# hpc4cmb/flacarray

Hardware: AMD Instinct MI355X
Metric: Msamples/s encode+decode, 4096ch x 1Msamp int32 (higher is better)
Workload: dtype int32

## Files before the change

flacarray_amd/csrc/decode_kernels.hpp:

```cpp
#pragma once
#include <hip/hip_runtime.h>
#include <stdint.h>

#include <type_traits>
#include <utility>

#include "flac_math.hpp"
#include "quantize_kernels.hpp"

namespace fa {

constexpr int kErrDecodeInit = 1 << 13;
constexpr int kErrDecodeProcess = 1 << 14;
constexpr int kErrDecodeSeek = 1 << 18;

constexpr int64_t kFrameUnset = -2;
constexpr int kScanSpan = 256 * 16;

struct StreamMeta {
    int64_t first_frame;
    int64_t seek_abs;
    int64_t end_abs;
    int32_t npoints;
    int32_t B;
// ... 372 lines not shown
            } else ok = false;
            if (ok && pred) {
                const int method = (int)br.get(2);
                const int po = (int)br.get(4);
                const int plen = method ? 5 : 4, esc = method ? 31 : 15;
                if (method > 1 || order > h.bs) ok = false;
                const int ps = h.bs >> po;
                for (int p = 0; ok && p < (1 << po); ++p) {
                    const int n = (p == 0) ? ps - order : ps;
                    if (n < 0) { ok = false; break; }
                    const int k = (int)br.get(plen);
                    if (k == esc) {
                        const int nbw = (int)br.get(5);
                        br.skip((int64_t)nbw * n);
                    } else {
                        for (int j = 0; j < n; ++j) {
                            const uint32_t q = br.unary();
                            if (q > (1u << 24)) { ok = false; break; }
                            if (k) br.get(k);
                        }
                    }
                }
            }
        }
        if (!ok) { atomicOr(err, kErrDecodeProcess); for (int64_t r = f + 1; r < nf; ++r) ftab[s * nf + r] = -1; return; }
        const int64_t bits = (br.used + 7) & ~(int64_t)7;
        at += (bits >> 3) + 2;
    }
    (void)stream_size;
}

struct DecodeArgs {
    const uint8_t* blob;
    int64_t blob_bytes;
    const StreamMeta* meta;
    const int64_t* ftab;
    int64_t nf;
    int32_t B;
    int64_t stream_size;
    int64_t n_tasks;
    int64_t nfr;
    int64_t f0;
    int64_t first;
    int64_t n_decode;
    const int64_t* task_stream;
    const int64_t* task_frame;
    const int64_t* task_first;
    const int64_t* task_last;
    const int64_t* task_out_off;
    union { int32_t* out_i32; long long* red_min; };
    union { float* out_f32; long long* red_max; };
    union { const float* offsets; long long* red_sum; };
    union { const float* gains; unsigned long long* red_sq_hi; };
    int* err;
    union { uint32_t* hibits; unsigned long long* red_sq_lo; };
    int32_t* assign;
    int32_t hib_words;
    int32_t verbatim_done;
    union { const void* cmp; int64_t red_width; };
    union { unsigned long long* first_mismatch; int64_t red_nbins; };
};

template <int... U, class F>
__device__ __forceinline__ void static_for_impl(std::integer_sequence<int, U...>, F&& f) {
    (f(std::integral_constant<int, U>{}), ...);
}
template <int N, class F>
__device__ __forceinline__ void static_for(F&& f) {
    static_for_impl(std::make_integer_sequence<int, N>{}, static_cast<F&&>(f));
}

#ifndef FA_TILE_W
#define FA_TILE_W 32
#endif
#ifndef FA_K7_SPEC
#define FA_K7_SPEC 0
#endif
#ifndef FA_K7_SEED
#define FA_K7_SEED 0
#endif
#ifndef FA_K7_NT
#define FA_K7_NT 1
#endif
#ifndef FA_K7_X
#define FA_K7_X 0
#endif
constexpr int kTileW = FA_TILE_W;
constexpr int kTileG = kTileW / 4;
constexpr int kTileSwz = 32 / kTileG;
#ifndef FA_CHUNK_BYTES
#define FA_CHUNK_BYTES 64
#endif
constexpr int kChunkBytes = FA_CHUNK_BYTES;
constexpr int kChunkW = kChunkBytes / 4;
constexpr int kChunkShift = (kChunkBytes == 64) ? 9 : 8;
constexpr int kRingW = 2 * kChunkW;
constexpr int kDecRingWords = kRingW + 2;
constexpr int kTopup = kChunkBytes / 8;
constexpr int kLaneStride = 64;

constexpr int kFlagNeed16 = 1, kFlagNeed32 = 2;
__device__ __forceinline__ int4 shl4(const int4& v, int n) {
    return make_int4((int)((uint32_t)v.x << n), (int)((uint32_t)v.y << n), (int)((uint32_t)v.z << n), (int)((uint32_t)v.w << n));
}

__device__ __forceinline__ void ring_load_chunk(const uint8_t* cbase, const uint8_t* lim16, uint32_t* ring, uint32_t ci) {
    const uint8_t* q = cbase + (size_t)ci * kChunkBytes;
    uint32_t* dst = ring + (ci & 1) * kChunkW * kLaneStride;
#pragma unroll
    for (int v = 0; v < kChunkBytes / 16; ++v) {
        uint4 d = make_uint4(0, 0, 0, 0);
        if (q + 16 * v + 16 <= lim16) d = *reinterpret_cast<const uint4*>(q + 16 * v);
        d.x = __builtin_bswap32(d.x); d.y = __builtin_bswap32(d.y); d.z = __builtin_bswap32(d.z); d.w = __builtin_bswap32(d.w);
        dst[(4 * v + 0) * kLaneStride] = d.x; dst[(4 * v + 1) * kLaneStride] = d.y;
        dst[(4 * v + 2) * kLaneStride] = d.z; dst[(4 * v + 3) * kLaneStride] = d.w;
        if (v == 0 && (ci & 1) == 0) { ring[kRingW * kLaneStride] = d.x; ring[(kRingW + 1) * kLaneStride] = d.y; }
    }
}
struct Chunk {
    uint4 d[kChunkBytes / 16];
};
__device__ __forceinline__ Chunk chunk_fetch(const uint8_t* cbase, const uint8_t* lim16, uint32_t ci) {
    const uint8_t* q = cbase + (size_t)ci * kChunkBytes;
    Chunk c;
#pragma unroll
    for (int v = 0; v < kChunkBytes / 16; ++v) {
        c.d[v] = make_uint4(0, 0, 0, 0);
#if (FA_K7_X & 8)
        c.d[v] = make_uint4(0x55555555u ^ ci, 0x55555555u, 0x55555555u, 0x55555555u);
#else
        if (q + 16 * v + 16 <= lim16) c.d[v] = *reinterpret_cast<const uint4*>(q + 16 * v);
#endif
    }
    return c;
}
__device__ __forceinline__ void chunk_store(uint32_t* ring, uint32_t ci, const Chunk& c) {
    uint32_t* dst = ring + (ci & 1) * kChunkW * kLaneStride;
#pragma unroll
    for (int v = 0; v < kChunkBytes / 16; ++v) {
        uint4 d = c.d[v];
        d.x = __builtin_bswap32(d.x); d.y = __builtin_bswap32(d.y); d.z = __builtin_bswap32(d.z); d.w = __builtin_bswap32(d.w);
        dst[(4 * v + 0) * kLaneStride] = d.x; dst[(4 * v + 1) * kLaneStride] = d.y;
        dst[(4 * v + 2) * kLaneStride] = d.z; dst[(4 * v + 3) * kLaneStride] = d.w;
        if (v == 0 && (ci & 1) == 0) { ring[kRingW * kLaneStride] = d.x; ring[(kRingW + 1) * kLaneStride] = d.y; }
    }
}
typedef __attribute__((address_space(3))) uint32_t lds_u32;
constexpr uint32_t kRingAddrMask = (uint32_t)(kRingW - 1) << 8;
__device__ __forceinline__ void ring_words(uint32_t lane4, uint32_t bitpos, uint32_t& w0, uint32_t& w1, uint32_t& w2) {
    static_assert(kLaneStride == 64, "word wi of a lane lies 256 wi bytes behind its word 0");
    uint32_t t, ad;
    asm("v_add_lshl_u32 %0, %2, -1, 3\n\tv_and_or_b32 %1, %0, %3, %4" : "=&v"(t), "=v"(ad) : "v"(bitpos), "s"(kRingAddrMask), "v"(lane4));
    const lds_u32* p = (const lds_u32*)(uintptr_t)ad;
    w0 = p[0]; w1 = p[kLaneStride]; w2 = p[2 * kLaneStride];
}
__device__ __forceinline__ uint32_t ring_word3(uint32_t lane4, uint32_t bitpos, uint32_t k95) {
    uint32_t t, ad;
    asm("v_add_lshl_u32 %0, %2, %5, 3\n\tv_and_or_b32 %1, %0, %3, %4" : "=&v"(t), "=v"(ad) : "v"(bitpos), "s"(kRingAddrMask), "v"(lane4), "s"(k95));
    return *(const lds_u32*)(uintptr_t)ad;
}
__device__ __forceinline__ void ring_window(const uint32_t* ring, uint32_t bitpos, uint32_t& A, uint32_t& B) {
    const uint32_t wi = (bitpos >> 5) & (kRingW - 1);
    const uint32_t off = bitpos & 31;
    uint32_t w0 = ring[wi * kLaneStride], w1 = ring[(wi + 1) * kLaneStride], w2 = ring[(wi + 2) * kLaneStride];
    asm volatile("" : "+v"(w0), "+v"(w1), "+v"(w2));
    A = (uint32_t)((((((uint64_t)w0) << 32) | w1) << off) >> 32);
// ... 65 lines not shown
        o.escw = r.val;
    }
    o.bitpos = r.bitpos;
    o.next_chunk = ring_ensure(cbase, lim16, ring, r.bitpos, r.next_chunk);
    return o;
}
__device__ __noinline__ BitsRet slow_sample(const uint8_t* cbase, const uint8_t* lim16, uint32_t* ring, uint32_t bitpos,
                                            uint32_t next_chunk, int k, int escw) {
    BitsRet r;
    if (escw > 0) {
        r = slow_get(cbase, lim16, ring, bitpos, next_chunk, escw);
        r.val = (uint32_t)((int32_t)(r.val << (32 - escw)) >> (32 - escw));
    } else {
        const BitsRet q = slow_unary(cbase, lim16, ring, bitpos, next_chunk);
        r = slow_get(cbase, lim16, ring, q.bitpos, q.next_chunk, k);
        const uint32_t uu = (q.val << k) | r.val;
        r.val = (uint32_t)((int32_t)(uu >> 1) ^ -(int32_t)(uu & 1));
        r.bad = q.bad;
    }
    r.next_chunk = ring_ensure(cbase, lim16, ring, r.bitpos, r.next_chunk);
    return r;
}

#define FA_GET(n) ({ const BitsRet r_ = slow_get(cbase, lim16, ring, bitpos, next_chunk, (n)); bitpos = r_.bitpos; next_chunk = r_.next_chunk; r_.val; })
#define FA_GETS(n) ({ const int n_ = (n); const uint32_t v_ = FA_GET(n_); (n_ == 0) ? 0 : ((int32_t)(v_ << (32 - n_)) >> (32 - n_)); })
#define FA_UNARY() ({ const BitsRet r_ = slow_unary(cbase, lim16, ring, bitpos, next_chunk); bitpos = r_.bitpos; next_chunk = r_.next_chunk; if (r_.bad) bad = true; r_.val; })

template <int MO, int MO_DONE, bool F32, int NCH, bool CMP = false, bool RED = false>
#ifndef FA_K7_WAVES_ATTR
#define FA_K7_WAVES_ATTR
#endif
__global__ __launch_bounds__(64) FA_K7_WAVES_ATTR void decode_frames_kernel(DecodeArgs a, int* flags) {
    constexpr int kTileW = (NCH == 1 && MO <= 16) ? FA_TILE_W : 32;
    constexpr int kTileG = kTileW / 4;
    constexpr int kTileSwz = 32 / kTileG;
    static_assert(NCH == 1 || (kTileW == 32 && !F32), "two-channel variant: 32-sample tiles, integer output");
    static_assert(!RED || (NCH == 1 && !F32 && !CMP), "reducing sink: one channel, integer domain");
    constexpr bool SINK = CMP && NCH == 1;
    __shared__ __attribute__((aligned(16))) uint32_t lds_k7[kDecRingWords * kLaneStride + (RED ? 0 : kTileW * kLaneStride) + (F32 ? 128 : 0)];
    uint32_t* const rings = lds_k7;
    int32_t* const tile = reinterpret_cast<int32_t*>(lds_k7 + kDecRingWords * kLaneStride);
    float2* const row_fg = reinterpret_cast<float2*>(lds_k7 + kDecRingWords * kLaneStride + kTileW * kLaneStride);
    const int lane = threadIdx.x;
    const int64_t task = (int64_t)blockIdx.x * 64 + lane;
    const bool has_task = task < a.n_tasks;
    uint32_t* const ring = rings + lane;
    const uint32_t lane4 = (uint32_t)(uintptr_t)(lds_u32*)ring;
    if ((uint32_t)(uintptr_t)(lds_u32*)rings & (kRingAddrMask | 255u)) {
        if (lane == 0) atomicOr(a.err, kErrDecodeInit);
        return;
    }

    int64_t s = 0, f = 0, sl_first = 0, sl_last = 0, out_off = 0;
    if (has_task) {
        if (a.task_stream) {
            s = a.task_stream[task]; f = a.task_frame[task];
            sl_first = a.task_first[task]; sl_last = a.task_last[task];
            out_off = a.task_out_off[task];
        } else {
            s = task / a.nfr; f = a.f0 + (task - s * a.nfr);
            sl_first = a.first; sl_last = a.first + a.n_decode;
            if constexpr (RED) out_off = s * a.red_nbins;
            else out_off = s * a.n_decode;
        }
    }
    const int64_t fstart = f * (int64_t)a.B;
    auto reject = [&]() __attribute__((always_inline)) {
        if constexpr (CMP) atomicMin(a.first_mismatch + s, (unsigned long long)fstart);
        else atomicOr(a.err, kErrDecodeProcess);
    };
    const uint8_t* cbase = a.blob;
    const uint8_t* const lim16 = reinterpret_cast<const uint8_t*>((reinterpret_cast<uintptr_t>(a.blob + a.blob_bytes) + 15) & ~(uintptr_t)15);
    uint32_t bitpos = 0, next_chunk = 0x00400000u;

    bool bad = false;
    bool task_live = has_task;
    int fbs = 0, fbps = 0, ch_assign = 0, si_bps = 0;
    if (has_task) {
        const StreamMeta m = a.meta[s];
        si_bps = m.bps;
        const int64_t at = a.ftab[s * a.nf + f];
        if (m.first_frame < 0 || at < 0) bad = true;
        else {
            const uint8_t* start = a.blob + at;
            cbase = reinterpret_cast<const uint8_t*>(reinterpret_cast<uintptr_t>(start - 1) & ~(uintptr_t)(kChunkBytes - 1));
            if (cbase < a.blob) cbase = a.blob;
            bitpos = (uint32_t)(start - cbase) * 8;
            ring_load_chunk(cbase, lim16, ring, 0);
            ring_load_chunk(cbase, lim16, ring, 1);
            next_chunk = 2;
            {
                uint8_t c8 = 0;
                const uint32_t w = FA_GET(32);
                c8 = crc8_byte(c8, (uint8_t)(w >> 24));
                c8 = crc8_byte(c8, (uint8_t)(w >> 16));
                c8 = crc8_byte(c8, (uint8_t)(w >> 8));
                c8 = crc8_byte(c8, (uint8_t)w);
                if ((w >> 16) != 0xFFF8) bad = true;
                const uint32_t b2 = (w >> 8) & 0xff, b3 = w & 0xff;
                const int bsc = (int)(b2 >> 4), src = (int)(b2 & 15), ch = (int)(b3 >> 4), ssc = (int)((b3 >> 1) & 7);
                if (!channel_code_ok(ch, NCH) || (b3 & 1)) bad = true;
                ch_assign = ch;
                const uint32_t u0 = FA_GET(8);
                c8 = crc8_byte(c8, (uint8_t)u0);
                int extra = 0;
                if (u0 & 0x80) {
                    int mbit = 0x40;
                    while ((u0 & mbit) && extra < 7) { extra++; mbit >>= 1; }
                    if (extra == 0 || extra > 6) bad = true;
                }
                for (int i = 0; i < extra && !bad; ++i) c8 = crc8_byte(c8, (uint8_t)FA_GET(8));
                if (bsc == 0) bad = true;
                else if (bsc == 1) fbs = 192;
                else if (bsc <= 5) fbs = 576 << (bsc - 2);
                else if (bsc == 6) { const uint32_t v = FA_GET(8); c8 = crc8_byte(c8, (uint8_t)v); fbs = (int)v + 1; }
                else if (bsc == 7) { const uint32_t v = FA_GET(16); c8 = crc8_byte(c8, (uint8_t)(v >> 8)); c8 = crc8_byte(c8, (uint8_t)v); fbs = (int)v + 1; }
                else fbs = 256 << (bsc - 8);
                if (src == 12) { c8 = crc8_byte(c8, (uint8_t)FA_GET(8)); }
                else if (src == 13 || src == 14) { const uint32_t v = FA_GET(16); c8 = crc8_byte(c8, (uint8_t)(v >> 8)); c8 = crc8_byte(c8, (uint8_t)v); }
                else if (src == 15) bad = true;
                if (FA_GET(8) != c8) bad = true;
                switch (ssc) {
                    case 0: fbps = si_bps; break;
                    case 1: fbps = 8; break;
                    case 2: fbps = 12; break;
                    case 4: fbps = 16; break;
                    case 5: fbps = 20; break;
                    case 6: fbps = 24; break;
                    case 7: fbps = 32; break;
                    default: bad = true; break;
                }
            }
            int64_t expect = a.stream_size - fstart;
            if (expect > a.B) expect = a.B;
            if (fbs != (int)expect) bad = true;
        }
        if constexpr (NCH == 2) {
            if (a.assign[task] >= 0) task_live = false;
        }
        if (bad) { task_live = false; reject(); }
    }
    const void* const out_base = SINK ? a.cmp : (a.out_f32 ? (const void*)a.out_f32 : (const void*)a.out_i32);
    const bool out_aligned = ((reinterpret_cast<uintptr_t>(out_base) & 15) == 0);

    auto get_wide = [&](int n) __attribute__((always_inline)) -> double {
        if constexpr (NCH == 2) {
            if (n > 32) {
                const uint32_t top = FA_GET(1);
                const uint32_t low = FA_GET(32);
                return (double)low - (top ? 4294967296.0 : 0.0);
            }
        }
        return (double)FA_GETS(n);
    };
    auto wrap32 = [&](double v) __attribute__((always_inline)) -> int32_t {
        if constexpr (NCH == 2) {
            if (v >= 2147483648.0) v -= 4294967296.0;
            else if (v < -2147483648.0) v += 4294967296.0;
        }
        return (int32_t)v;
    };

#pragma unroll 1
    for (int chn = 0; chn < NCH; ++chn) {
    int lo = 0, hi = 0;
    int bs = 0;
    int mode = 3;
    int order = 0, bps = 0, wasted = 0;
    double cval = 0.0;
    double scale = 1.0;
// ... 465 lines not shown
#endif
                } else {
#if (FA_K7_X & 2)
                    if (v.x == 0x12345678)
#endif
#if FA_K7_NT
                    {
                        typedef int i32x4_t __attribute__((ext_vector_type(4)));
                        i32x4_t vv; vv.x = v.x; vv.y = v.y; vv.z = v.z; vv.w = v.w;
                        __builtin_nontemporal_store(vv, reinterpret_cast<i32x4_t*>(a.out_i32 + rout[it] + tbase + cb));
                    }
#else
                    *reinterpret_cast<int4*>(a.out_i32 + rout[it] + tbase + cb) = v;
#endif
                }
            }
            __builtin_amdgcn_wave_barrier();
            return;
        }
#pragma unroll
        for (int it = 0; it < kTileG; ++it) {
            const int r = it * kRowsPerPass + (lane / kTileG);
            const int cg = lane % kTileG;
            const int cb = 4 * cg;
            const int rsw = r ^ (cg * kTileSwz);
            int4 v = make_int4(tile[(cb + 0) * kLaneStride + rsw], tile[(cb + 1) * kLaneStride + rsw], tile[(cb + 2) * kLaneStride + rsw],
                               tile[(cb + 3) * kLaneStride + rsw]);
            if (__builtin_expect(any_wasted, 0)) v = shl4(v, __builtin_amdgcn_ds_bpermute(r << 2, wasted));
            const int2 rg = make_int2(__builtin_amdgcn_ds_bpermute(r << 2, lo), __builtin_amdgcn_ds_bpermute(r << 2, hi));
            const int si = tbase + cb;
            int jd = 4;
            if (si + 3 >= rg.x && si < rg.y) {
                const int64_t ob = rout[it] + si;
                const bool fullv = (si >= rg.x) && (si + 3 < rg.y) && out_aligned && ((ob & 3) == 0);
                if constexpr (SINK) {
                    if (fullv) {
                        const int4 x = input4(ob, r);
                        jd = (v.x != x.x) ? 0 : (v.y != x.y) ? 1 : (v.z != x.z) ? 2 : (v.w != x.w) ? 3 : 4;
                    } else {
                        if (si + 3 >= rg.x && si + 3 < rg.y && input1(ob + 3, r) != v.w) jd = 3;
                        if (si + 2 >= rg.x && si + 2 < rg.y && input1(ob + 2, r) != v.z) jd = 2;
                        if (si + 1 >= rg.x && si + 1 < rg.y && input1(ob + 1, r) != v.y) jd = 1;
                        if (si + 0 >= rg.x && si + 0 < rg.y && input1(ob + 0, r) != v.x) jd = 0;
                    }
                } else if constexpr (F32) {
                    const float2 fg = row_fg[r];
                    float4 o;
                    o.x = __fadd_rn(fg.x, __fmul_rn(fg.y, (float)v.x));
                    o.y = __fadd_rn(fg.x, __fmul_rn(fg.y, (float)v.y));
                    o.z = __fadd_rn(fg.x, __fmul_rn(fg.y, (float)v.z));
                    o.w = __fadd_rn(fg.x, __fmul_rn(fg.y, (float)v.w));
                    if (fullv) *reinterpret_cast<float4*>(a.out_f32 + ob) = o;
                    else {
                        if (si + 0 >= rg.x && si + 0 < rg.y) a.out_f32[ob + 0] = o.x;
                        if (si + 1 >= rg.x && si + 1 < rg.y) a.out_f32[ob + 1] = o.y;
                        if (si + 2 >= rg.x && si + 2 < rg.y) a.out_f32[ob + 2] = o.z;
                        if (si + 3 >= rg.x && si + 3 < rg.y) a.out_f32[ob + 3] = o.w;
                    }
                } else {
                    if (fullv) *reinterpret_cast<int4*>(a.out_i32 + ob) = v;
                    else {
                        if (si + 0 >= rg.x && si + 0 < rg.y) a.out_i32[ob + 0] = v.x;
                        if (si + 1 >= rg.x && si + 1 < rg.y) a.out_i32[ob + 1] = v.y;
                        if (si + 2 >= rg.x && si + 2 < rg.y) a.out_i32[ob + 2] = v.z;
                        if (si + 3 >= rg.x && si + 3 < rg.y) a.out_i32[ob + 3] = v.w;
                    }
                }
            }
            if constexpr (SINK) report(r, rout[it] + si, jd);
        }
        __builtin_amdgcn_wave_barrier();
    };

    const int bs_max = a.B;
    constexpr int MACRO = kTileW;
    static_assert(MACRO % MO == 0 && MACRO % 16 == 0, "history rotation and tile must divide the macro step");
    auto macro_step = [&](auto guard_tag, auto part_tag, int i0) __attribute__((always_inline)) {
        static_for<MACRO>([&](auto ut) __attribute__((always_inline)) {
            constexpr int u = decltype(ut)::value;
            const int i = i0 + u;
            if constexpr ((u % kTopup) == 0) {
                topup();
            }
            sample(guard_tag, part_tag, ut, i);
            if constexpr (u == MACRO - 1) flush_tile(i0);
        });
    };
    constexpr int kStep = (MACRO > kTileW) ? MACRO : kTileW;
    int end = (bs_max + kStep - 1) / kStep * kStep;
    if (chn == NCH - 1) {
        const int need = (hi_max + kStep - 1) / kStep * kStep;
        if (need < end) end = need;
    }
    if constexpr (NCH == 2) {
        if (!__any(mode != 3)) end = 0;
    }
    int main_lo = (32 + MACRO - 1) / MACRO * MACRO;
    if (main_lo > end) main_lo = end;
    int main_hi = (bs_min < bs_max ? bs_min : bs_max) / MACRO * MACRO;
    if (main_hi > end) main_hi = end;
    if (main_hi < main_lo) main_hi = main_lo;
    for (int pass = 0; pass < 2; ++pass) {
        const int g_lo = pass == 0 ? 0 : main_hi;
        const int g_hi = pass == 0 ? main_lo : end;
        for (int i0 = g_lo; i0 < g_hi; i0 += MACRO) macro_step(std::true_type{}, std::true_type{}, i0);
        if (pass == 0) {
            for (int i0 = main_lo; i0 < main_hi; i0 += MACRO) {
                if (__any(pleft < MACRO)) {
                    macro_step(std::false_type{}, std::true_type{}, i0);
                } else {
                    macro_step(std::false_type{}, std::false_type{}, i0);
                    pleft -= MACRO;
                }
            }
        }
    }
    if constexpr (NCH == 2) {
        if (skipped) {
            bitpos = resume_bitpos;
            next_chunk = ring_ensure(cbase, lim16, ring, bitpos, bitpos >> kChunkShift);
        }
    }
    }
    if constexpr (NCH == 2) {
        if (has_task && task_live) a.assign[task] = ch_assign;
    }
}

__global__ __launch_bounds__(256) void verbatim_channel0_kernel(DecodeArgs a) {
    const int64_t task = blockIdx.x;
    int64_t s, f, sl_first, sl_last;
    if (a.task_stream) {
        s = a.task_stream[task]; f = a.task_frame[task];
        sl_first = a.task_first[task]; sl_last = a.task_last[task];
    } else {
        s = task / a.nfr; f = a.f0 + (task - s * a.nfr);
        sl_first = a.first; sl_last = a.first + a.n_decode;
    }
    const StreamMeta m = a.meta[s];
    const int64_t at = a.ftab[s * a.nf + f];
    if (m.first_frame < 0 || at < 0 || at + 5 > a.blob_bytes) return;
    const uint8_t* const p = a.blob + at;
    const uint32_t b2 = p[2], b3 = p[3], u0 = p[4];
    const int bsc = (int)(b2 >> 4), src = (int)(b2 & 15), ch = (int)(b3 >> 4), ssc = (int)((b3 >> 1) & 7);
    if (p[0] != 0xFF || p[1] != 0xF8 || (ch != 1 && ch != 8 && ch != 9 && ch != 10)) return;
    int extra = 0;
    if (u0 & 0x80) {
        int mbit = 0x40;
        while ((u0 & mbit) && extra < 7) { extra++; mbit >>= 1; }
        if (extra == 0 || extra > 6) return;
    }
    const int hl = 4 + 1 + extra + (bsc == 6 ? 1 : bsc == 7 ? 2 : 0) + (src == 12 ? 1 : (src == 13 || src == 14) ? 2 : 0) + 1;
    if (at + hl + 1 > a.blob_bytes || p[hl] != 0x02) return;
    int fbps;
    switch (ssc) {
        case 0: fbps = m.bps; break;
        case 1: fbps = 8; break;
        case 2: fbps = 12; break;
        case 4: fbps = 16; break;
        case 5: fbps = 20; break;
        case 6: fbps = 24; break;
        case 7: fbps = 32; break;
        default: return;
    }
    const int bps = fbps + (ch == 9 ? 1 : 0);
    if (bps <= 0 || bps > 33) return;
    const int64_t fstart = f * (int64_t)a.B;
    int64_t bs = a.stream_size - fstart;
    if (bs > a.B) bs = a.B;
    int64_t lo = sl_first - fstart, hi = sl_last - fstart;
    if (lo < 0) lo = 0;
    if (hi > bs) hi = bs;
    if (hi <= lo) return;
    int32_t* const t0 = a.out_i32 + (task * 2 + 0) * (int64_t)a.B;
    uint32_t* const h0 = a.hibits + (task * 2 + 0) * (int64_t)a.hib_words;
    const uint64_t bit0 = 8ull * (uint64_t)(hl + 1);
    const int lane = threadIdx.x & 63;
    const int64_t i0 = lo & ~(int64_t)31;
    const int64_t i1 = ((hi + 31) & ~(int64_t)31) < ((bs + 31) & ~(int64_t)31) ? ((hi + 31) & ~(int64_t)31) : ((bs + 31) & ~(int64_t)31);
    for (int64_t i = i0 + threadIdx.x; i < i1; i += 256) {
        uint32_t low = 0;
        bool neg = false;
        if (i < bs) {
            const uint64_t bp = bit0 + (uint64_t)i * (uint64_t)bps;
            const int64_t q = at + (int64_t)(bp >> 3);
            uint64_t w = 0;
            if (q + 8 <= a.blob_bytes) {
                uint32_t r0, r1;
                __builtin_memcpy(&r0, a.blob + q, 4);
                __builtin_memcpy(&r1, a.blob + q + 4, 4);
                w = ((uint64_t)__builtin_bswap32(r0) << 32) | __builtin_bswap32(r1);
            } else {
                for (int k = 0; k < 8; ++k) w = (w << 8) | (q + k < a.blob_bytes ? a.blob[q + k] : 0u);
            }
            const uint64_t v = (w << (bp & 7)) >> (64 - bps);
            neg = ((v >> (bps - 1)) & 1) != 0;
            low = (bps >= 32) ? (uint32_t)v : (uint32_t)((int32_t)((uint32_t)v << (32 - bps)) >> (32 - bps));
            if (i >= lo && i < hi) t0[i] = (int32_t)low;
        }
// ... 92 lines not shown
```

flacarray_amd/csrc/decode_latency.hpp:

```cpp
#pragma once
#include "decode_kernels.hpp"

namespace fa {

#ifndef FA_LAT_X
#define FA_LAT_X 0
#endif
#ifndef FA_LAT_SEG_BASE
#define FA_LAT_SEG_BASE 4
#endif
#ifndef FA_LAT_SEG_DIV
#define FA_LAT_SEG_DIV 36
#endif
#ifndef FA_LAT_STAMPS
#define FA_LAT_STAMPS 0
#endif
#if FA_LAT_STAMPS
#define FA_LAT_STAMP(i) do { lat_t[i] = __builtin_amdgcn_s_memrealtime(); } while (0)
#else
#define FA_LAT_STAMP(i) do { } while (0)
#endif
constexpr int kLatMaxBlock = 4096;
constexpr int kLatImgWords = 4416;
constexpr int kLatPadWords = 8;
// ... 42 lines not shown
    v += (uint32_t)__builtin_amdgcn_update_dpp(0, (int)v, 0x114, 0xF, 0xF, true);
    v += (uint32_t)__builtin_amdgcn_update_dpp(0, (int)v, 0x118, 0xF, 0xF, true);
    v += (uint32_t)__builtin_amdgcn_update_dpp(0, (int)v, 0x142, 0xA, 0xF, false);
    v += (uint32_t)__builtin_amdgcn_update_dpp(0, (int)v, 0x143, 0xC, 0xF, false);
    return v;
}
__device__ __forceinline__ void lat_restore_fixed(int32_t* res, int order, int hi) {
    const int lane = threadIdx.x & 63;
    uint32_t w[4] = {0u, 0u, 0u, 0u};
    for (int t = 0; t < order; ++t) w[t] = (uint32_t)res[order - 1 - t];
    for (int j = order - 1; j >= 0; --j) {
        uint32_t carry;
        if (j == 0) carry = w[0];
        else if (j == 1) carry = w[0] - w[1];
        else if (j == 2) carry = w[0] - 2u * w[1] + w[2];
        else carry = w[0] - 3u * w[1] + 3u * w[2] - w[3];
        for (int base = order; base < hi; base += 64) {
            const uint32_t s = lat_scan_incl_u32((uint32_t)res[base + lane]) + carry;
            res[base + lane] = (int32_t)s;
            carry = (uint32_t)__builtin_amdgcn_readlane((int)s, 63);
        }
    }
}

template <int K>
__device__ __forceinline__ void lat_lpc_step(double& acc, double c) {
    double x;
    asm volatile("s_nop 1\n\tv_floor_f64_dpp %0, %1 row_newbcast:%3 row_mask:0xf bank_mask:0xf\n\tv_fmac_f64 %1, %0, %2"
                 : "=&v"(x), "+v"(acc) : "v"(c), "n"(K));
}

__device__ __forceinline__ void lat_restore_lpc(int32_t* res, const double* coef16, int order, int hi) {
    const int m = threadIdx.x & 15;
    double cr[16];
#pragma unroll
    for (int k = 0; k < 16; ++k) cr[k] = coef16[(m - k - 1) & 15];
    int base = order;
    double acc = (double)res[base + m];
    for (int j = 0; j < order; ++j) {
        const int xi = base + m - 1 - j;
        if (xi < base) acc = __builtin_fma(coef16[j], (double)res[xi], acc);
    }
    const bool g0 = (m >> 2) == 0, g1 = (m >> 2) == 1, g2 = (m >> 2) == 2, g3 = (m >> 2) == 3;
    for (; base < hi; base += 16) {
        const double rn = (double)res[base + 16 + m];
        int32_t out = 0;
        auto hand_over = [&](bool mine) __attribute__((always_inline)) {
            const int32_t t = (int32_t)fa_floor(acc);
            out = mine ? t : out;
            acc = mine ? rn : acc;
        };
#define FA_LAT_STEP(K) lat_lpc_step<K>(acc, cr[K]);
        FA_LAT_STEP(0) FA_LAT_STEP(1) FA_LAT_STEP(2) FA_LAT_STEP(3)
        hand_over(g0);
        FA_LAT_STEP(4) FA_LAT_STEP(5) FA_LAT_STEP(6) FA_LAT_STEP(7)
        hand_over(g1);
        FA_LAT_STEP(8) FA_LAT_STEP(9) FA_LAT_STEP(10) FA_LAT_STEP(11)
        hand_over(g2);
        FA_LAT_STEP(12) FA_LAT_STEP(13) FA_LAT_STEP(14) FA_LAT_STEP(15)
        hand_over(g3);
#undef FA_LAT_STEP
        res[base + m] = out;
    }
}

struct LatWide {
    int64_t* out_i64;
    double* out_f64;
    const double* offsets;
    const double* gains;
};

template <bool F32, int NCH>
__global__ __launch_bounds__(64) void decode_latency_kernel(DecodeArgs a, LatInline inl, LatWide wd, int* fallback) {
    constexpr int kImgWords = (NCH == 2) ? kLatImgWords2 : kLatImgWords;
    constexpr uint32_t kTop = (NCH == 2) ? kLatTop2 : kLatTop;
    __shared__ __attribute__((aligned(16))) uint32_t img[kImgWords + kLatPadWords];
    __shared__ __attribute__((aligned(16))) int32_t res_all[NCH][kLatMaxBlock + kLatResPad];
    __shared__ double coef_s[16];
    const int lane = threadIdx.x;
    const int64_t task = blockIdx.x;
    if (task >= a.n_tasks) return;
    auto give_up = [&](int why) __attribute__((always_inline)) {
        if (lane == 0) *reinterpret_cast<volatile int*>(fallback) = why;
    };

#if FA_LAT_STAMPS
    uint64_t lat_t[8] = {0, 0, 0, 0, 0, 0, 0, 0};
    uint32_t lat_rounds = 0, lat_parts = 0, lat_segs = 0, lat_codes = 0, lat_k = 0, lat_S = 0;
#endif
    FA_LAT_STAMP(0);
    int64_t s, f, sl_first, sl_last, out_off;
    if (inl.n > 0) {
        s = inl.stream[task]; f = inl.frame[task]; sl_first = inl.first[task]; sl_last = inl.last[task]; out_off = inl.out_off[task];
    } else if (a.task_stream) {
        s = a.task_stream[task]; f = a.task_frame[task];
        sl_first = a.task_first[task]; sl_last = a.task_last[task];
        out_off = a.task_out_off[task];
    } else {
        s = task / a.nfr; f = a.f0 + (task - s * a.nfr);
        sl_first = a.first; sl_last = a.first + a.n_decode;
        out_off = s * a.n_decode;
    }
    const StreamMeta m = a.meta[s];
    const int64_t at = a.ftab[s * a.nf + f];
    const int64_t nxt = (f + 1 < a.nf) ? a.ftab[s * a.nf + f + 1] : m.end_abs;
    if (m.first_frame < 0 || at < 0 || nxt <= at + 6 || nxt > a.blob_bytes || a.B > kLatMaxBlock || m.channels != NCH) { give_up(1); return; }
    const int64_t base = at & ~(int64_t)15;
    const uint32_t skip = (uint32_t)(at - base);
    const uint32_t nbytes = skip + (uint32_t)(nxt - at);
    if (nbytes > (uint32_t)kImgWords * 4u) { give_up(1); return; }
    const uint32_t frame_end_bits = nbytes * 8u;

    {
        const uint32_t pieces = (nbytes + 15u) >> 4;
        const uint8_t* const q0 = a.blob + base;
        for (uint32_t i0 = 0; i0 < pieces; i0 += 512) {
            uint4 d[8];
#pragma unroll
            for (int t = 0; t < 8; ++t) {
                uint32_t i = i0 + 64u * (uint32_t)t + (uint32_t)lane;
                i = i < pieces ? i : pieces - 1u;
                d[t] = *reinterpret_cast<const uint4*>(q0 + 16 * (int64_t)i);
            }
#pragma unroll
            for (int t = 0; t < 8; ++t) {
                const uint32_t i = i0 + 64u * (uint32_t)t + (uint32_t)lane;
                if (i < pieces) {
                    uint4 o;
                    o.w = __builtin_bswap32(d[t].x); o.z = __builtin_bswap32(d[t].y); o.y = __builtin_bswap32(d[t].z); o.x = __builtin_bswap32(d[t].w);
                    *reinterpret_cast<uint4*>(&img[kTop - 3u - 4u * i]) = o;
                }
            }
        }
        for (uint32_t i = 4 * pieces + lane; i < (uint32_t)(kImgWords + kLatPadWords); i += 64) img[kTop - i] = 0;
    }
    __syncthreads();
    FA_LAT_STAMP(1);

    uint32_t pos = skip * 8u;
    bool bad = false;
    auto get = [&](int n) __attribute__((always_inline)) -> uint32_t {
        if (pos + (uint32_t)n > frame_end_bits) { bad = true; return 0u; }
        const uint32_t v = lat_win<kTop>(img, pos) >> (32 - n);
        pos += (uint32_t)n;
        return v;
    };
    auto gets = [&](int n) __attribute__((always_inline)) -> int32_t {
        if (n == 0) return 0;
        const uint32_t v = get(n);
        return (int32_t)(v << (32 - n)) >> (32 - n);
    };

    int bs = 0, fbps = 0, assign = 0;
    {
        uint8_t c8 = 0;
        const uint32_t w = get(32);
        c8 = crc8_byte(c8, (uint8_t)(w >> 24)); c8 = crc8_byte(c8, (uint8_t)(w >> 16));
        c8 = crc8_byte(c8, (uint8_t)(w >> 8)); c8 = crc8_byte(c8, (uint8_t)w);
        if ((w >> 16) != 0xFFF8) bad = true;
        const uint32_t b2 = (w >> 8) & 0xff, b3 = w & 0xff;
        const int bsc = (int)(b2 >> 4), src = (int)(b2 & 15), ch = (int)(b3 >> 4), ssc = (int)((b3 >> 1) & 7);
        if constexpr (NCH == 2) {
            if ((ch != 1 && ch != 8 && ch != 9) || (b3 & 1)) bad = true;
            assign = ch;
        } else {
            if (ch != 0 || (b3 & 1)) bad = true;
// ... 326 lines not shown
```

flacarray_amd/csrc/splice_kernels.hpp:

```cpp
#pragma once
#include <hip/hip_runtime.h>
#include <stdint.h>

#include "decode_kernels.hpp"
#include "encode_placed.hpp"

namespace fa {

FA_HD uint32_t crc16_mulmod(uint32_t a, uint32_t b) {
    uint32_t p = 0;
    for (int i = 0; i < 16; ++i)
        if ((b >> i) & 1u) p ^= a << i;
    for (int i = 31; i >= 16; --i)
        if ((p >> i) & 1u) p ^= 0x18005u << (i - 16);
    return p;
}
FA_HD uint32_t crc16_xpow8(uint64_t n) {
    uint32_t r = 1, b = 0x100;
    while (n) {
        if (n & 1) r = crc16_mulmod(r, b);
        b = crc16_mulmod(b, b);
        n >>= 1;
    }
    return r;
// ... 31 lines not shown
    int64_t n_stream, m, size_old, size_new, f0, f1, nf_old, nf_new;
    int32_t B, nch, parts;
};

__device__ __forceinline__ int64_t splice_nfe(const SpliceArgs& a) { return a.nf_new - a.f0 - (a.nf_old - a.f1); }

__device__ __forceinline__ bool old_stream_kept(const SpliceArgs& a, int64_t s, int64_t frame, int64_t* kept) {
    const int64_t hb_old = stream_header_bytes(a.nf_old);
    const int64_t os = a.old_starts[s], on = a.old_nbytes[s];
    *kept = 0;
    if (os < 0 || on < hb_old || os + on > a.old_bytes) return false;
    const uint8_t* h = a.old + os;
    const uint32_t stl = ((uint32_t)h[43] << 16) | ((uint32_t)h[44] << 8) | h[45];
    const uint64_t packed = load_be64(h + 18);
    const uint64_t total = ((uint64_t)a.size_old < (1ULL << 36)) ? (uint64_t)a.size_old : 0;
    if (h[0] != 'f' || h[1] != 'L' || h[2] != 'a' || h[3] != 'C' || h[4] != 0 || h[42] != 0x83 || stl != 18u * (uint32_t)a.nf_old ||
        h[8] != (uint8_t)(a.B >> 8) || h[9] != (uint8_t)a.B || (int)((packed >> 41) & 7u) + 1 != a.nch ||
        (packed & ((1ULL << 36) - 1)) != total)
        return false;
    const int64_t k = (frame < a.nf_old) ? (int64_t)load_be64(h + 46 + 18 * frame + 8) : on - hb_old;
    if (k < 0 || k > on - hb_old) return false;
    *kept = k;
    return true;
}

__device__ __forceinline__ bool splice_bounds(const SpliceArgs& a, int64_t s, int64_t* o0, int64_t* o1) {
    const bool ok0 = old_stream_kept(a, s, a.f0, o0);
    const bool ok1 = old_stream_kept(a, s, a.f1, o1);
    return ok0 && ok1 && *o0 <= *o1;
}

__device__ __forceinline__ int64_t splice_row(const SpliceArgs& a, int64_t s) { return a.sidx ? (int64_t)a.slot[s] : s; }

__global__ __launch_bounds__(256) void splice_check_kernel(SpliceArgs a) {
    const int64_t j = (int64_t)blockIdx.x * 256 + threadIdx.x;
    if (j >= a.m) return;
    int64_t s = j;
    a.sub_starts[j] = 0;
    a.sub_nbytes[j] = 0;
    if (a.sidx) {
        s = a.sidx[j];
        if (s < 0 || s >= a.n_stream || atomicExch(&a.slot[s], (int32_t)j) != -1) {
            atomicOr(a.err, 4);
            return;
        }
    }
    int64_t o0, o1;
    if (!splice_bounds(a, s, &o0, &o1)) {
        atomicOr(a.err, 2);
        return;
    }
    a.sub_starts[j] = a.old_starts[s];
    a.sub_nbytes[j] = a.old_nbytes[s];
}

__global__ __launch_bounds__(256) void splice_size_kernel(SpliceArgs a) {
    const int64_t s = (int64_t)blockIdx.x * 256 + threadIdx.x;
    if (s >= a.n_stream) return;
    const int64_t os = a.old_starts[s], on = a.old_nbytes[s];
    const int64_t j = splice_row(a, s);
    int64_t o0 = 0, o1 = 0, size = on;
    if (j < 0) {
        if (os < 0 || on < 0 || os + on > a.old_bytes) {
            atomicOr(a.err, 2);
            size = 0;
        }
    } else {
        const int64_t nfe = splice_nfe(a);
        const int64_t hb_enc = stream_header_bytes(nfe);
        const int64_t es = a.enc_starts[j], en = a.enc_nbytes[j];
        if (!splice_bounds(a, s, &o0, &o1) || es < 0 || en < hb_enc || es + en > a.enc_bytes) {
            atomicOr(a.err, 2);
            o0 = o1 = 0;
            size = 0;
        } else {
            size = on + (stream_header_bytes(a.nf_new) - stream_header_bytes(a.nf_old)) - (o1 - o0) + (en - hb_enc) + append_growth(a.f0, nfe);
        }
    }
    a.off0[s] = o0;
    a.off1[s] = o1;
    a.nbytes[s] = size;
}

__device__ __forceinline__ uint4 funnel16(const uint8_t* s, uint32_t q) {
    const uint8_t* blk = s - q;
    const uint4 lo = *reinterpret_cast<const uint4*>(blk);
    if (q == 0) return lo;
    const uint4 hi = *reinterpret_cast<const uint4*>(blk + 16);
    const uint32_t sh = q & 3u;
    uint32_t w0, w1, w2, w3, w4;
    switch (q >> 2) {
        case 0: w0 = lo.x; w1 = lo.y; w2 = lo.z; w3 = lo.w; w4 = hi.x; break;
        case 1: w0 = lo.y; w1 = lo.z; w2 = lo.w; w3 = hi.x; w4 = hi.y; break;
        case 2: w0 = lo.z; w1 = lo.w; w2 = hi.x; w3 = hi.y; w4 = hi.z; break;
        default: w0 = lo.w; w1 = hi.x; w2 = hi.y; w3 = hi.z; w4 = hi.w; break;
    }
    return make_uint4(__builtin_amdgcn_alignbyte(w1, w0, sh), __builtin_amdgcn_alignbyte(w2, w1, sh), __builtin_amdgcn_alignbyte(w3, w2, sh),
                      __builtin_amdgcn_alignbyte(w4, w3, sh));
}

__device__ void copy_segment(uint8_t* __restrict__ dst, const uint8_t* __restrict__ src, int64_t len, const uint8_t* src_end, int64_t t,
                             int64_t nthr) {
    if (len <= 0) return;
    const uintptr_t d0 = reinterpret_cast<uintptr_t>(dst), d1 = d0 + (uintptr_t)len;
    const uintptr_t c0 = d0 & ~(uintptr_t)15, c1 = (d1 + 15) & ~(uintptr_t)15;
    const int64_t nchunk = (int64_t)((c1 - c0) >> 4);
    const int64_t delta = reinterpret_cast<intptr_t>(src) - reinterpret_cast<intptr_t>(dst);
    const uint32_t q = (uint32_t)(((uintptr_t)src - (uintptr_t)dst) & 15u);
    constexpr int U = 4;
    for (int64_t i0 = t; i0 < nchunk; i0 += U * nthr) {
        uint4 v[U];
        bool full[U];
#pragma unroll
        for (int u = 0; u < U; ++u) {
            const int64_t i = i0 + (int64_t)u * nthr;
            const uintptr_t c = c0 + ((uintptr_t)i << 4);
            const uint8_t* s = reinterpret_cast<const uint8_t*>((intptr_t)c + delta);
            full[u] = i < nchunk && c >= d0 && c + 16 <= d1 && (s - q) + (q ? 32 : 16) <= src_end;
            if (full[u]) v[u] = funnel16(s, q);
        }
#pragma unroll
        for (int u = 0; u < U; ++u) {
            const int64_t i = i0 + (int64_t)u * nthr;
            if (i >= nchunk) break;
            const uintptr_t c = c0 + ((uintptr_t)i << 4);
            if (full[u]) {
                *reinterpret_cast<uint4*>(c) = v[u];
            } else {
                for (int b = 0; b < 16; ++b) {
                    const uintptr_t d = c + (uintptr_t)b;
                    if (d >= d0 && d < d1) *reinterpret_cast<uint8_t*>(d) = *reinterpret_cast<const uint8_t*>((intptr_t)d + delta);
                }
            }
        }
    }
}

__device__ __forceinline__ void renumber_frame_wave(uint8_t* fd, const uint8_t* fr, int64_t L, uint64_t v, const uint8_t* src_end, int lane) {
    uint32_t hw0 = 0, hw1 = 0, hw2 = 0, hw3 = 0, crc_new = 0;
    int h_old = 0, h_new = 0;
    if (lane == 0) {
        const uint8_t lead = fr[4];
        int u = 0;
        while (u < 7 && (lead & (0x80u >> u))) ++u;
        u = u ? u : 1;
        const int code = fr[2] >> 4;
        const int extra = (code == 6) ? 1 : (code == 7) ? 2 : 0;
        h_old = 4 + u + extra + 1;
        const int un = utf8_bytes(v);
        auto setb = [&](int i, uint32_t b8) {
            const uint32_t sh = 8u * (uint32_t)(i & 3), m = ~(0xFFu << sh), b = (b8 & 0xFFu) << sh;
            if (i < 4) hw0 = (hw0 & m) | b; else if (i < 8) hw1 = (hw1 & m) | b; else if (i < 12) hw2 = (hw2 & m) | b; else hw3 = (hw3 & m) | b;
        };
        auto getb = [&](int i) -> uint8_t {
            const uint32_t w = (i < 4) ? hw0 : (i < 8) ? hw1 : (i < 12) ? hw2 : hw3;
            return (uint8_t)(w >> (8 * (i & 3)));
        };
        for (int i = 0; i < 4; ++i) setb(i, fr[i]);
        if (un == 1) {
            setb(4, (uint32_t)v);
        } else {
            setb(4, ((0xFF00u >> un) & 0xFFu) | (uint32_t)(v >> (6 * (un - 1))));
            for (int i = 1; i < un; ++i) setb(4 + i, 0x80u | (uint32_t)((v >> (6 * (un - 1 - i))) & 0x3Fu));
        }
        for (int i = 0; i < extra; ++i) setb(4 + un + i, fr[4 + u + i]);
        h_new = 4 + un + extra + 1;
        uint8_t c8 = 0;
        uint16_t ch_old = 0, ch_new = 0;
        for (int i = 0; i < h_new - 1; ++i) c8 = crc8_byte(c8, getb(i));
        setb(h_new - 1, c8);
        for (int i = 0; i < h_old; ++i) ch_old = crc16_byte(ch_old, fr[i]);
        for (int i = 0; i < h_new; ++i) ch_new = crc16_byte(ch_new, getb(i));
        const uint32_t crc_old = ((uint32_t)fr[L - 2] << 8) | fr[L - 1];
        crc_new = crc_old ^ crc16_mulmod((uint32_t)(ch_old ^ ch_new), crc16_xpow8((uint64_t)(L - 2 - h_old)));
    }
    h_old = __shfl(h_old, 0, 64);
    h_new = __shfl(h_new, 0, 64);
    hw0 = (uint32_t)__shfl((int)hw0, 0, 64);
    hw1 = (uint32_t)__shfl((int)hw1, 0, 64);
    hw2 = (uint32_t)__shfl((int)hw2, 0, 64);
    hw3 = (uint32_t)__shfl((int)hw3, 0, 64);
    if (lane < h_new) {
        const uint32_t w = (lane < 4) ? hw0 : (lane < 8) ? hw1 : (lane < 12) ? hw2 : hw3;
        fd[lane] = (uint8_t)(w >> (8 * (lane & 3)));
    }
    copy_segment(fd + h_new, fr + h_old, L - 2 - h_old, src_end, lane, 64);
    if (lane == 0) {
        fd[h_new + L - 2 - h_old] = (uint8_t)(crc_new >> 8);
        fd[h_new + L - 1 - h_old] = (uint8_t)crc_new;
    }
}

__device__ __forceinline__ void store_be64(uint8_t* p, uint64_t v) {
#pragma unroll
    for (int i = 0; i < 8; ++i) p[i] = (uint8_t)(v >> (56 - 8 * i));
}

__global__ __launch_bounds__(256) void splice_kernel(SpliceArgs a) {
    const int64_t s = (int64_t)blockIdx.x / a.parts;
    const int p = (int)((int64_t)blockIdx.x - s * a.parts);
    const int tid = threadIdx.x;
    const int64_t t = (int64_t)p * 256 + tid, nthr = (int64_t)a.parts * 256;
    uint8_t* const dst = a.out + a.starts[s];
    const uint8_t* const osrc = a.old + a.old_starts[s];
    const uint8_t* const old_end = a.old + a.old_bytes;
    const int64_t on = a.old_nbytes[s];
    const int64_t j = splice_row(a, s);
    if (j < 0) {
        copy_segment(dst, osrc, on, old_end, t, nthr);
        return;
    }
    const int64_t nfe = splice_nfe(a);
    const int64_t hb = stream_header_bytes(a.nf_new), hb_old = stream_header_bytes(a.nf_old), hb_enc = stream_header_bytes(nfe);
    const uint8_t* const esrc = a.enc + a.enc_starts[j];
// ... 36 lines not shown
```

Measured before the change: 207,700.

## Defer tile flush by one macro step and use global address space pointers

The decode sample loop now flushes the previous tile at the start of the next macro step instead of at the end of the current one, so the store of one tile can overlap with decoding of the next. A final flush after the loops handles the last tile. Separately, the splice copy and the latency fallback write now use explicit address_space(1) pointers so the compiler can emit global rather than flat memory instructions. The chunk base computation is also rewritten as integer offsets relative to the blob's alignment. The deferred flush relies on tile contents staying intact until the next step, which adds register or LDS lifetime pressure.

```diff
diff --git a/flacarray_amd/csrc/decode_kernels.hpp b/flacarray_amd/csrc/decode_kernels.hpp
--- a/flacarray_amd/csrc/decode_kernels.hpp
+++ b/flacarray_amd/csrc/decode_kernels.hpp
@@ -478,6 +478,9 @@
 #ifndef FA_K7_NT
 #define FA_K7_NT 1
 #endif
+#ifndef FA_K7_LATE_FLUSH
+#define FA_K7_LATE_FLUSH 1
+#endif
 #ifndef FA_K7_X
 #define FA_K7_X 0
 #endif
@@ -709,10 +712,11 @@
         const int64_t at = a.ftab[s * a.nf + f];
         if (m.first_frame < 0 || at < 0) bad = true;
         else {
-            const uint8_t* start = a.blob + at;
-            cbase = reinterpret_cast<const uint8_t*>(reinterpret_cast<uintptr_t>(start - 1) & ~(uintptr_t)(kChunkBytes - 1));
-            if (cbase < a.blob) cbase = a.blob;
-            bitpos = (uint32_t)(start - cbase) * 8;
+            const int64_t mis = (int64_t)(reinterpret_cast<uintptr_t>(a.blob) & (uintptr_t)(kChunkBytes - 1));
+            int64_t coff = ((at - 1 + mis) & ~(int64_t)(kChunkBytes - 1)) - mis;
+            if (coff < 0) coff = 0;
+            cbase = a.blob + coff;
+            bitpos = (uint32_t)(at - coff) * 8;
             ring_load_chunk(cbase, lim16, ring, 0);
             ring_load_chunk(cbase, lim16, ring, 1);
             next_chunk = 2;
@@ -1344,8 +1348,15 @@
             if constexpr ((u % kTopup) == 0) {
                 topup();
             }
+#if FA_K7_LATE_FLUSH
+            if constexpr (u == 0) {
+                if (i0 > 0) flush_tile(i0 - MACRO);
+            }
+#endif
             sample(guard_tag, part_tag, ut, i);
+#if !FA_K7_LATE_FLUSH
             if constexpr (u == MACRO - 1) flush_tile(i0);
+#endif
         });
     };
     constexpr int kStep = (MACRO > kTileW) ? MACRO : kTileW;
@@ -1377,6 +1388,9 @@
             }
         }
     }
+#if FA_K7_LATE_FLUSH
+    if (end > 0) flush_tile(end - MACRO);
+#endif
     if constexpr (NCH == 2) {
         if (skipped) {
             bitpos = resume_bitpos;
diff --git a/flacarray_amd/csrc/decode_latency.hpp b/flacarray_amd/csrc/decode_latency.hpp
--- a/flacarray_amd/csrc/decode_latency.hpp
+++ b/flacarray_amd/csrc/decode_latency.hpp
@@ -148,7 +148,7 @@
     const int64_t task = blockIdx.x;
     if (task >= a.n_tasks) return;
     auto give_up = [&](int why) __attribute__((always_inline)) {
-        if (lane == 0) *reinterpret_cast<volatile int*>(fallback) = why;
+        if (lane == 0) *(volatile __attribute__((address_space(1))) int*)fallback = why;
     };
 
 #if FA_LAT_STAMPS
diff --git a/flacarray_amd/csrc/splice_kernels.hpp b/flacarray_amd/csrc/splice_kernels.hpp
--- a/flacarray_amd/csrc/splice_kernels.hpp
+++ b/flacarray_amd/csrc/splice_kernels.hpp
@@ -137,11 +137,14 @@
     a.nbytes[s] = size;
 }
 
-__device__ __forceinline__ uint4 funnel16(const uint8_t* s, uint32_t q) {
-    const uint8_t* blk = s - q;
-    const uint4 lo = *reinterpret_cast<const uint4*>(blk);
-    if (q == 0) return lo;
-    const uint4 hi = *reinterpret_cast<const uint4*>(blk + 16);
+typedef __attribute__((address_space(1))) uint8_t g_u8;
+typedef uint32_t g_u32x4_t __attribute__((ext_vector_type(4)));
+typedef __attribute__((address_space(1))) g_u32x4_t g_u32x4;
+__device__ __forceinline__ uint4 funnel16(const g_u8* s, uint32_t q) {
+    const g_u8* blk = s - q;
+    const g_u32x4_t lo = *reinterpret_cast<const g_u32x4*>(blk);
+    if (q == 0) return make_uint4(lo.x, lo.y, lo.z, lo.w);
+    const g_u32x4_t hi = *reinterpret_cast<const g_u32x4*>(blk + 16);
     const uint32_t sh = q & 3u;
     uint32_t w0, w1, w2, w3, w4;
     switch (q >> 2) {
@@ -157,10 +160,13 @@
 __device__ void copy_segment(uint8_t* __restrict__ dst, const uint8_t* __restrict__ src, int64_t len, const uint8_t* src_end, int64_t t,
                              int64_t nthr) {
     if (len <= 0) return;
+    g_u8* const gd = (g_u8*)dst;
+    const g_u8* const gs = (const g_u8*)src;
+    const g_u8* const gend = (const g_u8*)src_end;
     const uintptr_t d0 = reinterpret_cast<uintptr_t>(dst), d1 = d0 + (uintptr_t)len;
     const uintptr_t c0 = d0 & ~(uintptr_t)15, c1 = (d1 + 15) & ~(uintptr_t)15;
     const int64_t nchunk = (int64_t)((c1 - c0) >> 4);
-    const int64_t delta = reinterpret_cast<intptr_t>(src) - reinterpret_cast<intptr_t>(dst);
+    const int64_t e0 = -(int64_t)(d0 & 15);
     const uint32_t q = (uint32_t)(((uintptr_t)src - (uintptr_t)dst) & 15u);
     constexpr int U = 4;
     for (int64_t i0 = t; i0 < nchunk; i0 += U * nthr) {
@@ -169,22 +175,24 @@
 #pragma unroll
         for (int u = 0; u < U; ++u) {
             const int64_t i = i0 + (int64_t)u * nthr;
-            const uintptr_t c = c0 + ((uintptr_t)i << 4);
-            const uint8_t* s = reinterpret_cast<const uint8_t*>((intptr_t)c + delta);
-            full[u] = i < nchunk && c >= d0 && c + 16 <= d1 && (s - q) + (q ? 32 : 16) <= src_end;
+            const int64_t o = e0 + (i << 4);
+            const g_u8* s = gs + o;
+            full[u] = i < nchunk && o >= 0 && o + 16 <= len && (s - q) + (q ? 32 : 16) <= gend;
             if (full[u]) v[u] = funnel16(s, q);
         }
 #pragma unroll
         for (int u = 0; u < U; ++u) {
             const int64_t i = i0 + (int64_t)u * nthr;
             if (i >= nchunk) break;
-            const uintptr_t c = c0 + ((uintptr_t)i << 4);
+            const int64_t o = e0 + (i << 4);
             if (full[u]) {
-                *reinterpret_cast<uint4*>(c) = v[u];
+                g_u32x4_t w;
+                w.x = v[u].x; w.y = v[u].y; w.z = v[u].z; w.w = v[u].w;
+                *reinterpret_cast<g_u32x4*>(gd + o) = w;
             } else {
                 for (int b = 0; b < 16; ++b) {
-                    const uintptr_t d = c + (uintptr_t)b;
-                    if (d >= d0 && d < d1) *reinterpret_cast<uint8_t*>(d) = *reinterpret_cast<const uint8_t*>((intptr_t)d + delta);
+                    const int64_t d = o + b;
+                    if (d >= 0 && d < len) gd[d] = gs[d];
                 }
             }
         }
```

Measured after the change: 211,400, median of 6. 1.8% higher.
